# ucsdmanorlab/PSSR2

Hardware: AMD Instinct MI355X
Metric: HR tiles/sec (512^2 4xSR) train (higher is better)
Workload: dtype bf16

## Files before the change

### include/pssr_mi355.h

```cpp
#ifndef PSSR_MI355_H
#define PSSR_MI355_H

#include <stdint.h>

#ifdef __cplusplus
extern "C" {
#endif

typedef void* pssr_stream_t;

enum { PSSR_F32 = 0, PSSR_BF16 = 1, PSSR_F16 = 2 };

enum {
    PSSR_OK = 0,
    PSSR_ERR_ARG = -1,
    PSSR_ERR_LAUNCH = -2,
    PSSR_ERR_UNSUPPORTED = -3
};

int pssr_abi_version(void);
const char* pssr_last_error(void);

int pssr_pack_conv_weight(const float* w_oihw, void* packed, int cout, int cin, int ks,
                          int ci_begin, int ci_count, int mode, const int32_t* n_perm,
// ... 133 lines not shown
                                  pssr_stream_t stream);

int pssr_channel_sum_nhwc(const void* x, int cs, int co, int64_t npix, int c, double* out, int dtype,
                          pssr_stream_t stream);
int pssr_nchw_to_nhwc(const float* in, void* out, int n, int c, int64_t hw, int out_cs, float scale,
                      int dtype, pssr_stream_t stream);
int pssr_clip_u8(const float* in, uint8_t* out, int64_t n, pssr_stream_t stream);
int pssr_f64_to_f32(const double* in, float* out, int n, int accumulate, int stripes, pssr_stream_t stream);

int pssr_ssim_level_fwd(const float* x, const float* y, int planes, int h, int w, const float* win_host,
                        int k, float c1, float c2, double* sums, double* l1_sum, pssr_stream_t stream);
int pssr_avgpool2_planes(const float* in, float* out, int planes, int h, int w, pssr_stream_t stream);
int pssr_msssim_weights(const double* sums, int levels, int planes, const double* nvalid,
                        const float* level_weights, int ms, float mix, const double* l1_sum,
                        double l1_numel, const float* grad_out, float* loss_out, float* wts,
                        float* l1_coef, pssr_stream_t stream);
int pssr_ssim_level_bwd(const float* x, const float* y, int planes, int h, int w, const float* win_host,
                        int k, float c1, float c2, const float* wts, int use_ssim, const float* dcoarse,
                        int hc, int wc, const float* l1_coef, float* dx, pssr_stream_t stream);

int pssr_ssim_level_fwd_adj(const float* x, const float* y, float in_div, int planes, int h, int w, const float* win_host, int k,
                            float c1, float c2, int use_ssim, double* sums, double* l1_sum, int stripes, int64_t stripe_stride,
                            float* adj, pssr_stream_t stream);
int pssr_msssim_weights_striped(const double* sums, int stripes, int64_t stripe_stride, double* folded, int levels, int planes,
                                const double* nvalid, const float* level_weights, int ms, float mix, const double* l1_sum,
                                double l1_numel, const float* grad_out, float* loss_out, float* wts, float* l1_coef,
                                pssr_stream_t stream);
int pssr_ssim_level_bwd_adj(const float* x, const float* y, float in_div, const float* adj, int planes, int h, int w,
                            const float* win_host, int k, const float* wts, const float* dcoarse, int hc, int wc,
                            const float* l1_coef, float* dx, pssr_stream_t stream);
int pssr_avgpool2_planes_div(const float* in, float in_div, float* out, int planes, int h, int w, pssr_stream_t stream);
int pssr_avgpool2_pair_div(const float* x, const float* y, float in_div, float* xo, float* yo, int planes, int h, int w,
                           pssr_stream_t stream);

int pssr_adamw_step(float* p, const float* g, float* m, float* v, int64_t n, float lr, float beta1,
                    float beta2, float eps, float weight_decay, int64_t step, float grad_scale,
                    pssr_stream_t stream);
int pssr_adamw_step_dev(float* p, const float* g, float* m, float* v, int64_t n, int64_t* state,
                        float beta1, float beta2, float eps, float weight_decay, float grad_scale,
                        pssr_stream_t stream);
int pssr_amp_check(const float* g, int64_t n, int32_t* amp, pssr_stream_t stream);
int pssr_adamw_step_amp(float* p, const float* g, float* m, float* v, int64_t n, int64_t* state,
                        float beta1, float beta2, float eps, float weight_decay, float grad_scale,
                        int32_t* amp, float growth, float backoff, int interval, pssr_stream_t stream);

int pssr_bilinear_down_u8(const uint8_t* hr, uint8_t* tmp, uint8_t* lr, int planes, int H, int W,
                          int h, int w, pssr_stream_t stream);
int pssr_u8_to_f32(const uint8_t* in, float* out, int64_t n, pssr_stream_t stream);
int pssr_crappify_gaussian(const float* in, float* out, int tiles, int64_t per_tile, float intensity,
                           float gain, float spread, uint64_t seed, uint64_t tile_offset,
                           const double* noise, int flags, const uint64_t* tile_counter,
                           pssr_stream_t stream);
int pssr_crappify_poisson(const float* in, float* out, int tiles, int64_t per_tile, float intensity,
                          float gain, float spread, uint64_t seed, uint64_t tile_offset, int flags,
                          const uint64_t* tile_counter, pssr_stream_t stream);
int pssr_crappify_poisson_samples(const float* in, const double* samples, float* out, int64_t n, double intensity,
                                  double gain, int flags, pssr_stream_t stream);
int pssr_counter_add(uint64_t* counter, uint64_t inc, pssr_stream_t stream);
int pssr_gaussian_blur(const float* in, float* tmp, float* out, int planes, int h, int w, float sigma,
                       float gain, int flags, pssr_stream_t stream);

int pssr_crappify_saltpepper(const float* in, float* out, int tiles, int64_t per_tile, float amount, float gain, float spread,
                             uint64_t seed, uint64_t tile_offset, int flags, const uint64_t* tile_counter, pssr_stream_t stream);
int pssr_gaussian_blur_tiles(const float* in, float* tmp, float* out, int tiles, int planes_per_tile, int h, int w, float sigma,
                             float spread, float gain, uint64_t seed, uint64_t tile_offset, int flags, const uint64_t* tile_counter,
                             pssr_stream_t stream);
// ... 148 lines not shown
```

### pssr2_amd/csrc/loss.hip

```cpp
#include "common.h"

namespace {

constexpr int TS = 32;
constexpr int MAXW = 33;

struct Win { float g[MAXW]; int k; };

template <int K_DUMMY>
__global__ __launch_bounds__(256) void ssim_fwd_kernel(const float* __restrict__ X, const float* __restrict__ Y, int H, int W,
                                                       Win win, float C1, float C2, double* sums ,
                                                       double* l1_sum ) {
    extern __shared__ float lds[];
    const int k = win.k, halo = k - 1, IN = TS + halo;
    float* xs = lds;
    float* ys = xs + IN * IN;
    float* hp = ys + IN * IN;
    const int plane = blockIdx.z;
    const int oy0 = blockIdx.y * TS, ox0 = blockIdx.x * TS;
    const int VH = H - halo, VW = W - halo;
    const float* xp = X + (long)plane * H * W;
    const float* yp = Y + (long)plane * H * W;
    const int tid = threadIdx.x;
    float l1 = 0.f;
// ... 340 lines not shown
        float v[5][SEG + K - 1];
#pragma unroll
        for (int q = 0; q < 5; ++q)
#pragma unroll
            for (int j = 0; j < SEG + K - 1; ++j) v[q][j] = hp[q * IN * HPW + (r0 + j) * HPW + c];
        float m[5][SEG];
        fir_seg<K, SEG, 5>(v, win, m);
#pragma unroll
        for (int j = 0; j < SEG; ++j) {
            if (oy0 + r0 + j >= VH || ox0 + c >= VW) continue;
            const float mx = m[0][j], my = m[1][j];
            const float sxx = m[2][j] - mx * mx, syy = m[3][j] - my * my, sxy = m[4][j] - mx * my;
            const float Dcs = sxx + syy + C2;
            const float cs = (2.f * sxy + C2) / Dcs;
            const float Dl = mx * mx + my * my + C1;
            const float lum = (2.f * mx * my + C1) / Dl;
            cs_acc += cs; ss_acc += lum * cs;
        }
    }
    __shared__ float red[3][256];
    red[0][tid] = cs_acc; red[1][tid] = ss_acc; red[2][tid] = l1;
    __syncthreads();
    for (int o = 128; o > 0; o >>= 1) {
        if (tid < o) { red[0][tid] += red[0][tid + o]; red[1][tid] += red[1][tid + o]; red[2][tid] += red[2][tid + o]; }
        __syncthreads();
    }
    if (tid == 0) {
        atomicAdd(sums + plane * 2, (double)red[0][0]);
        atomicAdd(sums + plane * 2 + 1, (double)red[1][0]);
        if (l1_sum) atomicAdd(l1_sum, (double)red[2][0]);
    }
}

template <int K>
__global__ __launch_bounds__(256) void ssim_fwd_adj_k(const float* __restrict__ X, const float* __restrict__ Y, int H, int W,
                                                      Win win, float C1, float C2, double* sums, double* l1_sum, int stripes, long stripe_stride,
                                                      float* __restrict__ adj, int use_ssim, float in_mul) {
    constexpr int halo = K - 1, IN = TS + halo, SEG = 8, NS = TS / SEG;
    constexpr int HPW = TS + 1;
    extern __shared__ float lds[];
    float* xs = lds;
    float* ys = xs + IN * IN;
    float* hp = ys + IN * IN;
    const int plane = blockIdx.z;
    const int oy0 = blockIdx.y * TS, ox0 = blockIdx.x * TS;
    const int VH = H - halo, VW = W - halo;
    const float* xp = X + (long)plane * H * W;
    const float* yp = Y + (long)plane * H * W;
    const int tid = threadIdx.x;
    float l1 = 0.f;
    for (int i = tid; i < IN * IN; i += 256) {
        const int r = i / IN, c = i % IN;
        const int gy = oy0 + r, gx = ox0 + c;
        float xv = 0.f, yv = 0.f;
        if (gy < H && gx < W) { xv = __fmul_rn(xp[(long)gy * W + gx], in_mul); yv = __fmul_rn(yp[(long)gy * W + gx], in_mul); }
        xs[i] = xv; ys[i] = yv;
    }
    __syncthreads();
    if (l1_sum) {
        constexpr int r5 = K / 2;
        float wsum = 0.f;
#pragma unroll
        for (int t = 0; t < K; ++t) wsum += win.g[t];
        for (int i = tid; i < TS * TS; i += 256) {
            const int r = i / TS, c = i % TS;
            const int gy = oy0 + r, gx = ox0 + c;
            if (gy < H && gx < W) {
                float sy = wsum, sx = wsum;
                if (gy < r5 || gy >= H - r5) {
                    sy = 0.f;
#pragma unroll
                    for (int t = 0; t < K; ++t) { const int yy = gy + t - r5; if (yy >= 0 && yy < H) sy += win.g[t]; }
                }
                if (gx < r5 || gx >= W - r5) {
                    sx = 0.f;
#pragma unroll
                    for (int t = 0; t < K; ++t) { const int xx = gx + t - r5; if (xx >= 0 && xx < W) sx += win.g[t]; }
                }
                l1 += fabsf(xs[r * IN + c] - ys[r * IN + c]) * sy * sx;
            }
        }
    }
    const bool vitem = tid < TS * NS;
    const int vc = tid % TS, vr0 = (tid / TS) * SEG;
    float m[5][SEG];
#pragma unroll
    for (int q = 0; q < 5; ++q) {
        for (int it = tid; it < IN * NS; it += 256) {
            const int r = it / NS, c0 = (it % NS) * SEG;
            float v[1][SEG + K - 1];
#pragma unroll
            for (int j = 0; j < SEG + K - 1; ++j) {
                const float a = (q == 1 || q == 3) ? 0.f : xs[r * IN + c0 + j];
                const float b = (q == 0 || q == 2) ? 0.f : ys[r * IN + c0 + j];
                v[0][j] = q == 0 ? a : q == 1 ? b : q == 2 ? a * a : q == 3 ? b * b : a * b;
            }
            float o[1][SEG];
            fir_seg<K, SEG, 1>(v, win, o);
#pragma unroll
            for (int j = 0; j < SEG; ++j) hp[r * HPW + c0 + j] = o[0][j];
        }
        __syncthreads();
        if (vitem) {
            float v[1][SEG + K - 1];
#pragma unroll
            for (int j = 0; j < SEG + K - 1; ++j) v[0][j] = hp[(vr0 + j) * HPW + vc];
            float o[1][SEG];
            fir_seg<K, SEG, 1>(v, win, o);
#pragma unroll
            for (int j = 0; j < SEG; ++j) m[q][j] = o[0][j];
        }
        if (q < 4) __syncthreads();
    }
    float cs_acc = 0.f, ss_acc = 0.f;
    if (vitem) {
#pragma unroll
        for (int j = 0; j < SEG; ++j) {
            if (oy0 + vr0 + j >= VH || ox0 + vc >= VW) continue;
            const float mx = m[0][j], my = m[1][j];
            const float sxx = m[2][j] - mx * mx, syy = m[3][j] - my * my, sxy = m[4][j] - mx * my;
            const float Dcs = sxx + syy + C2;
            const float cs = (2.f * sxy + C2) / Dcs;
            const float Dl = mx * mx + my * my + C1;
            const float lum = (2.f * mx * my + C1) / Dl;
            cs_acc += cs; ss_acc += lum * cs;
            const float dcs_dmx = 2.f * (cs * mx - my) / Dcs, dcs_dexx = -cs / Dcs, dcs_dexy = 2.f / Dcs;
            float a = dcs_dmx, b = dcs_dexx, cc = dcs_dexy;
            if (use_ssim) {
                const float dl_dmx = 2.f * (my - lum * mx) / Dl;
                a = lum * dcs_dmx + cs * dl_dmx; b = lum * dcs_dexx; cc = lum * dcs_dexy;
            }
            float* ap = adj + ((long)plane * 3 * H + (oy0 + vr0 + j)) * W + ox0 + vc;
            ap[0] = a; ap[(long)H * W] = b; ap[2L * H * W] = cc;
        }
    }
    __shared__ float red[3][256];
    red[0][tid] = cs_acc; red[1][tid] = ss_acc; red[2][tid] = l1;
    __syncthreads();
    for (int o = 128; o > 0; o >>= 1) {
        if (tid < o) { red[0][tid] += red[0][tid + o]; red[1][tid] += red[1][tid + o]; red[2][tid] += red[2][tid + o]; }
        __syncthreads();
    }
    if (tid == 0) {
        const long so = (long)((blockIdx.x + blockIdx.y * 5) % stripes) * stripe_stride, lo = (long)stripes * stripe_stride;
        stat_add(sums + so + plane * 2, lo, red[0][0]);
        stat_add(sums + so + plane * 2 + 1, lo, red[1][0]);
        if (l1_sum) stat_add(l1_sum + so, lo, red[2][0]);
    }
}

template <int K>
__global__ __launch_bounds__(256) void ssim_bwd_adj_k(const float* __restrict__ X, const float* __restrict__ Y, const float* __restrict__ ADJ,
                                                      int H, int W, Win win, const float* __restrict__ wts,
                                                      const float* __restrict__ dcoarse, int HC, int WC, const float* l1_coef_p,
                                                      float* __restrict__ dX, float in_mul) {
    constexpr int halo = K - 1, AD = TS + halo;
    constexpr int SEG = 8, NS = TS / SEG;
    constexpr int ADC = AD + 1;
    constexpr int THR = AD + SEG, THW = TS + 1;
    constexpr int NL = (AD * AD + 255) / 256;
    extern __shared__ float lds[];
    float* ad = lds;
    float* th = lds + AD * ADC;
    const int plane = blockIdx.z;
    const int qy0 = blockIdx.y * TS, qx0 = blockIdx.x * TS;
    const int VH = H - halo, VW = W - halo;
    const float* xp = X + (long)plane * H * W;
    const float* yp = Y + (long)plane * H * W;
    const float* ap = ADJ + (long)plane * 3 * H * W;
    const int tid = threadIdx.x;
    const float wt = wts[plane];
    int goff[NL], lslot[NL];
#pragma unroll
    for (int u = 0; u < NL; ++u) {
        const int i = tid + u * 256;
        const int r = i / AD, c = i - r * AD;
        const int py = qy0 - halo + r, px = qx0 - halo + c;
        lslot[u] = i < AD * AD ? r * ADC + c : -1;
        goff[u] = (i < AD * AD && py >= 0 && py < VH && px >= 0 && px < VW) ? py * W + px : -1;
    }
    float pre[NL];
#define SB_LOAD(Q)                                                                                                \
    _Pragma("unroll") for (int u = 0; u < NL; ++u) pre[u] = goff[u] >= 0 ? wt * ap[(long)(Q) * H * W + goff[u]] : 0.f;
    SB_LOAD(0)
    const bool vitem = tid < TS * NS;
    const int vc = tid % TS, vr0 = (tid / TS) * SEG;
    float xv[SEG], yv[SEG], gsum[SEG];
#pragma unroll
    for (int o = 0; o < SEG; ++o) {
        const int gy = qy0 + vr0 + o, gx = qx0 + vc;
        const bool ok = vitem && gy < H && gx < W;
        xv[o] = ok ? __fmul_rn(xp[(long)gy * W + gx], in_mul) : 0.f;
        yv[o] = ok ? __fmul_rn(yp[(long)gy * W + gx], in_mul) : 0.f;
        gsum[o] = 0.f;
    }
#pragma unroll
    for (int q = 0; q < 3; ++q) {
#pragma unroll
        for (int u = 0; u < NL; ++u) if (lslot[u] >= 0) ad[lslot[u]] = pre[u];
        __syncthreads();
        if (q < 2) { SB_LOAD(q + 1) }
        for (int it = tid; it < AD * NS; it += 256) {
            const int r = it / NS, c0 = (it % NS) * SEG;
            float v[SEG + K - 1];
#pragma unroll
            for (int j = 0; j < SEG + K - 1; ++j) v[j] = ad[r * ADC + c0 + j];
#pragma unroll
            for (int o = 0; o < SEG; ++o) {
                float s_ = 0.f;
#pragma unroll
                for (int t = 0; t < K; ++t) s_ = fmaf(win.g[t], v[o + halo - t], s_);
                th[r * THW + c0 + o] = s_;
            }
        }
        __syncthreads();
        if (vitem) {
            float v[SEG + K - 1];
#pragma unroll
            for (int j = 0; j < SEG + K - 1; ++j) v[j] = th[(vr0 + j) * THW + vc];
#pragma unroll
            for (int o = 0; o < SEG; ++o) {
                float a = 0.f;
#pragma unroll
                for (int t = 0; t < K; ++t) a = fmaf(win.g[t], v[o + halo - t], a);
                if (q == 0) gsum[o] = a;
                else if (q == 1) gsum[o] = gsum[o] + 2.f * xv[o] * a;
                else gsum[o] = gsum[o] + yv[o] * a;
            }
        }
    }
#undef SB_LOAD
    if (!vitem) return;
    const float l1c = l1_coef_p ? l1_coef_p[0] : 0.f;
    constexpr int r5 = K / 2;
    float wsum = 0.f;
#pragma unroll
    for (int t = 0; t < K; ++t) wsum += win.g[t];
    float* dxp = dX + (long)plane * H * W;
#pragma unroll
    for (int o = 0; o < SEG; ++o) {
        const int gy = qy0 + vr0 + o, gx = qx0 + vc;
        if (gy >= H || gx >= W) continue;
        float g = gsum[o];
        if (dcoarse) {
            const int cy = (gy + (H & 1)) >> 1, cx = (gx + (W & 1)) >> 1;
            g += 0.25f * dcoarse[((long)plane * HC + cy) * WC + cx];
        }
        if (l1c != 0.f) {
            float sy = wsum, sx = wsum;
            if (gy < r5 || gy >= H - r5) {
                sy = 0.f;
#pragma unroll
                for (int t = 0; t < K; ++t) { const int yy = gy + t - r5; if (yy >= 0 && yy < H) sy += win.g[t]; }
            }
            if (gx < r5 || gx >= W - r5) {
                sx = 0.f;
#pragma unroll
                for (int t = 0; t < K; ++t) { const int xx = gx + t - r5; if (xx >= 0 && xx < W) sx += win.g[t]; }
            }
            const float d = xv[o] - yv[o];
            g += l1c * sy * sx * (d > 0.f ? 1.f : (d < 0.f ? -1.f : 0.f));
        }
        dxp[(long)gy * W + gx] = __fmul_rn(g, in_mul);
    }
}

template <int K>
__global__ __launch_bounds__(256, 2) void ssim_bwd_k(const float* __restrict__ X, const float* __restrict__ Y, int H, int W, Win win,
                                                  float C1, float C2, const float* __restrict__ wts, int use_ssim,
                                                  const float* __restrict__ dcoarse, int HC, int WC, const float* l1_coef_p,
                                                  float* __restrict__ dX) {
    constexpr int halo = K - 1, AD = TS + halo, IN = TS + 2 * halo;
    constexpr int SA = 7, NSA = (AD + SA - 1) / SA;
    constexpr int SEG = 8, NS = TS / SEG;
    constexpr int ADP = NSA * SA;
    extern __shared__ float lds[];
    float* xs = lds;
    constexpr int INP = IN + SA;
    float* ys = xs + IN * INP;
    float* hp = ys + IN * INP;
    float* ad = lds;
    constexpr int ADR = AD, ADC = AD;
    static_assert(3 * AD * AD <= 2 * IN * INP, "adjoint maps must fit into the input images");
    const int plane = blockIdx.z;
    const int qy0 = blockIdx.y * TS, qx0 = blockIdx.x * TS;
    const int VH = H - halo, VW = W - halo;
    const float* xp = X + (long)plane * H * W;
    const float* yp = Y + (long)plane * H * W;
    const int tid = threadIdx.x;
    const float wt = wts[plane];
    for (int i = tid; i < IN * INP; i += 256) {
        const int r = i / INP, c = i % INP;
        const int gy = qy0 - halo + r, gx = qx0 - halo + c;
        float xv = 0.f, yv = 0.f;
        if (c < IN && gy >= 0 && gy < H && gx >= 0 && gx < W) { xv = xp[(long)gy * W + gx]; yv = yp[(long)gy * W + gx]; }
        xs[i] = xv; ys[i] = yv;
    }
// ... 139 lines not shown
int pssr_ssim_level_fwd(const float* x, const float* y, int planes, int h, int w, const float* win_host, int k,
                        float c1, float c2, double* sums, double* l1_sum, pssr_stream_t s) {
    PSSR_CHECK(x && y && sums && win_host && planes > 0 && k > 0 && k <= MAXW && (k & 1), PSSR_ERR_ARG, "ssim_level_fwd: bad args");
    PSSR_CHECK(h >= k && w >= k, PSSR_ERR_ARG, "ssim_level_fwd: image %dx%d smaller than window %d", h, w, k);
    const int IN = TS + k - 1;
    const size_t lds = (size_t)(2 * IN * IN + 5 * IN * (TS + 1)) * sizeof(float);
    const int eh = l1_sum ? h : h - k + 1, ew = l1_sum ? w : w - k + 1;
    static bool attr = false;
    if (!attr) {
        (void)hipFuncSetAttribute((const void*)ssim_fwd_kernel<0>, hipFuncAttributeMaxDynamicSharedMemorySize, 160 * 1024 - 4096);
        (void)hipFuncSetAttribute((const void*)ssim_fwd_k<11>, hipFuncAttributeMaxDynamicSharedMemorySize, 160 * 1024 - 4096);
        attr = true;
    }
    if (k == 11)
        hipLaunchKernelGGL(ssim_fwd_k<11>, dim3(cdiv(ew, TS), cdiv(eh, TS), planes), dim3(256), lds, (hipStream_t)s, x, y, h, w,
                           make_win(win_host, k), c1, c2, sums, l1_sum);
    else
        hipLaunchKernelGGL(ssim_fwd_kernel<0>, dim3(cdiv(ew, TS), cdiv(eh, TS), planes), dim3(256), lds, (hipStream_t)s, x, y, h, w,
                           make_win(win_host, k), c1, c2, sums, l1_sum);
    PSSR_LAUNCH_CHECK();
    return PSSR_OK;
}

int pssr_ssim_level_fwd_adj(const float* x, const float* y, float in_div, int planes, int h, int w, const float* win_host, int k, float c1,
                            float c2, int use_ssim, double* sums, double* l1_sum, int stripes, int64_t stripe_stride, float* adj,
                            pssr_stream_t s) {
    PSSR_CHECK(x && y && sums && win_host && planes > 0 && adj && k == 11, PSSR_ERR_ARG,
               "ssim_level_fwd_adj: needs the adjoint buffer and the 11-tap window (k=%d)", k);
    PSSR_CHECK(h >= k && w >= k && stripes >= 1 && (stripes == 1 || stripe_stride > 0) && in_div > 0.f, PSSR_ERR_ARG, "ssim_level_fwd_adj: bad size / stripes / in_div");
    const int IN = TS + k - 1;
    const size_t lds = (size_t)(2 * IN * IN + IN * (TS + 1)) * sizeof(float);
    const int eh = l1_sum ? h : h - k + 1, ew = l1_sum ? w : w - k + 1;
    hipLaunchKernelGGL(ssim_fwd_adj_k<11>, dim3(cdiv(ew, TS), cdiv(eh, TS), planes), dim3(256), lds, (hipStream_t)s, x, y, h, w,
                       make_win(win_host, k), c1, c2, sums, l1_sum, stripes, (long)stripe_stride, adj, use_ssim, in_div == 1.f ? 1.f : 1.f / in_div);
    PSSR_LAUNCH_CHECK();
    return PSSR_OK;
}

int pssr_ssim_level_bwd_adj(const float* x, const float* y, float in_div, const float* adj, int planes, int h, int w, const float* win_host,
                            int k, const float* wts, const float* dcoarse, int hc, int wc, const float* l1_coef, float* dx, pssr_stream_t s) {
    PSSR_CHECK(x && y && adj && wts && dx && win_host && planes > 0 && k == 11, PSSR_ERR_ARG, "ssim_level_bwd_adj: bad args (k=%d)", k);
    constexpr int AD = TS + 10;
    const size_t lds = (size_t)(AD * (AD + 1) + (AD + 8) * (TS + 1)) * sizeof(float);
    hipLaunchKernelGGL(ssim_bwd_adj_k<11>, dim3(cdiv(w, TS), cdiv(h, TS), planes), dim3(256), lds, (hipStream_t)s, x, y, adj, h, w,
                       make_win(win_host, k), wts, dcoarse, hc, wc, l1_coef, dx, in_div == 1.f ? 1.f : 1.f / in_div);
    PSSR_LAUNCH_CHECK();
    return PSSR_OK;
}

int pssr_avgpool2_planes(const float* in, float* out, int planes, int h, int w, pssr_stream_t s) {
    return pssr_avgpool2_planes_div(in, 1.f, out, planes, h, w, s);
}

int pssr_avgpool2_planes_div(const float* in, float in_div, float* out, int planes, int h, int w, pssr_stream_t s) {
    PSSR_CHECK(in && out && planes > 0 && h > 0 && w > 0 && in_div > 0.f, PSSR_ERR_ARG, "avgpool2_planes: bad args");
    const int ho = (h + 2 * (h & 1) - 2) / 2 + 1, wo = (w + 2 * (w & 1) - 2) / 2 + 1;
    const long total = (long)planes * ho * wo;
    int blocks = (int)((total + 255) / 256); if (blocks > 8192) blocks = 8192;
    hipLaunchKernelGGL(avgpool_kernel, dim3(blocks), dim3(256), 0, (hipStream_t)s, in, out, in, out, planes, h, w, ho, wo, in_div == 1.f ? 1.f : 1.f / in_div);
    PSSR_LAUNCH_CHECK();
    return PSSR_OK;
}

int pssr_avgpool2_pair_div(const float* x, const float* y, float in_div, float* xo, float* yo, int planes, int h, int w, pssr_stream_t s) {
    PSSR_CHECK(x && y && xo && yo && planes > 0 && h > 0 && w > 0 && in_div > 0.f, PSSR_ERR_ARG, "avgpool2_pair: bad args");
    const int ho = (h + 2 * (h & 1) - 2) / 2 + 1, wo = (w + 2 * (w & 1) - 2) / 2 + 1;
    const long total = (long)planes * ho * wo;
    int blocks = (int)((total + 255) / 256); if (blocks > 8192) blocks = 8192;
    hipLaunchKernelGGL(avgpool_kernel, dim3(blocks, 2), dim3(256), 0, (hipStream_t)s, x, xo, y, yo, planes, h, w, ho, wo, in_div == 1.f ? 1.f : 1.f / in_div);
    PSSR_LAUNCH_CHECK();
    return PSSR_OK;
}

int pssr_msssim_weights(const double* sums, int levels, int planes, const double* nvalid, const float* level_weights, int ms,
                        float mix, const double* l1_sum, double l1_numel, const float* grad_out, float* loss_out, float* wts,
                        float* l1_coef, pssr_stream_t s) {
    PSSR_CHECK(sums && nvalid && loss_out && wts && l1_coef && levels > 0 && levels <= 8 && planes > 0, PSSR_ERR_ARG, "msssim_weights: bad args");
    hipLaunchKernelGGL(weights_kernel, dim3(1), dim3(256), 0, (hipStream_t)s, sums, levels, planes, nvalid, level_weights, ms, mix,
// ... 41 lines not shown
```

### pssr2_amd/ops.py

```python
from __future__ import annotations

import ctypes as C

import torch

from . import _lib as L

TORCH_DTYPE = {L.F32: torch.float32, L.BF16: torch.bfloat16, L.F16: torch.float16}


def dtype_code(dt: torch.dtype) -> int:
    if dt == torch.float32:
        return L.F32
    if dt == torch.bfloat16:
        return L.BF16
    if dt == torch.float16:
        return L.F16
    raise ValueError(f"unsupported compute dtype {dt}; use torch.float32, torch.bfloat16 or torch.float16")


def pad_to(v: int, m: int) -> int:
    return (v + m - 1) // m * m


# ... 220 lines not shown


def _win(win):
    arr = (C.c_float * len(win))(*[float(v) for v in win])
    return arr, len(win)


def ssim_level_fwd(x, y, planes, h, w, win, c1, c2, sums, l1_sum=None):
    arr, k = _win(win)
    L.check(L.lib().pssr_ssim_level_fwd(L.ptr(x), L.ptr(y), planes, h, w, arr, k, C.c_float(c1), C.c_float(c2), L.ptr(sums),
                                        L.ptr(l1_sum), L.stream_ptr()), "pssr_ssim_level_fwd")


def ssim_level_fwd_adj(x, y, planes, h, w, win, c1, c2, use_ssim, sums, l1_sum, stripes, stripe_stride, adj, in_div=1.0):
    k = len(win); arr = (C.c_float * k)(*win)
    L.check(L.lib().pssr_ssim_level_fwd_adj(L.ptr(x), L.ptr(y), C.c_float(in_div), planes, h, w, arr, k, C.c_float(c1), C.c_float(c2), int(use_ssim), L.ptr(sums),
                                            L.ptr(l1_sum), stripes, C.c_int64(stripe_stride), L.ptr(adj), L.stream_ptr()), "pssr_ssim_level_fwd_adj")


def msssim_weights_striped(sums, stripes, stripe_stride, folded, levels, planes, nvalid, level_weights, ms, mix, l1_sum, l1_numel, grad_out,
                           loss_out, wts, l1_coef):
    L.check(L.lib().pssr_msssim_weights_striped(L.ptr(sums), stripes, C.c_int64(stripe_stride), L.ptr(folded), levels, planes, L.ptr(nvalid),
                                                L.ptr(level_weights), int(ms), C.c_float(mix), L.ptr(l1_sum), C.c_double(l1_numel),
                                                L.ptr(grad_out), L.ptr(loss_out), L.ptr(wts), L.ptr(l1_coef), L.stream_ptr()),
            "pssr_msssim_weights_striped")


def ssim_level_bwd_adj(x, y, adj, planes, h, w, win, wts, dcoarse, hc, wc, l1_coef, dx, in_div=1.0):
    k = len(win); arr = (C.c_float * k)(*win)
    L.check(L.lib().pssr_ssim_level_bwd_adj(L.ptr(x), L.ptr(y), C.c_float(in_div), L.ptr(adj), planes, h, w, arr, k, L.ptr(wts), L.ptr(dcoarse), hc, wc,
                                            L.ptr(l1_coef), L.ptr(dx), L.stream_ptr()), "pssr_ssim_level_bwd_adj")


def avgpool2_planes(x, out, planes, h, w, in_div=1.0):
    L.check(L.lib().pssr_avgpool2_planes_div(L.ptr(x), C.c_float(in_div), L.ptr(out), planes, h, w, L.stream_ptr()), "pssr_avgpool2_planes_div")


def avgpool2_pair(x, y, xo, yo, planes, h, w, in_div=1.0):
    L.check(L.lib().pssr_avgpool2_pair_div(L.ptr(x), L.ptr(y), C.c_float(in_div), L.ptr(xo), L.ptr(yo), planes, h, w, L.stream_ptr()),
            "pssr_avgpool2_pair_div")


def msssim_weights(sums, levels, planes, nvalid, level_weights, ms, mix, l1_sum, l1_numel, grad_out, loss_out, wts, l1_coef):
    L.check(L.lib().pssr_msssim_weights(L.ptr(sums), levels, planes, L.ptr(nvalid), L.ptr(level_weights), int(ms), C.c_float(mix),
                                        L.ptr(l1_sum), C.c_double(l1_numel), L.ptr(grad_out), L.ptr(loss_out), L.ptr(wts),
                                        L.ptr(l1_coef), L.stream_ptr()), "pssr_msssim_weights")


def ssim_level_bwd(x, y, planes, h, w, win, c1, c2, wts, use_ssim, dcoarse, hc, wc, l1_coef, dx):
    arr, k = _win(win)
    L.check(L.lib().pssr_ssim_level_bwd(L.ptr(x), L.ptr(y), planes, h, w, arr, k, C.c_float(c1), C.c_float(c2), L.ptr(wts),
                                        int(use_ssim), L.ptr(dcoarse), hc, wc, L.ptr(l1_coef), L.ptr(dx), L.stream_ptr()),
            "pssr_ssim_level_bwd")


def adamw_step(p, g, m, v, lr, beta1, beta2, eps, weight_decay, step, grad_scale=1.0):
    L.check(L.lib().pssr_adamw_step(L.ptr(p), L.ptr(g), L.ptr(m), L.ptr(v), C.c_int64(p.numel()), C.c_float(lr), C.c_float(beta1),
                                    C.c_float(beta2), C.c_float(eps), C.c_float(weight_decay), C.c_int64(step), C.c_float(grad_scale),
                                    L.stream_ptr()), "pssr_adamw_step")


ROUND_CLIP, CLIP = 2, 1


def bilinear_down_u8(hr, h, w):
    assert hr.dtype == torch.uint8 and hr.is_cuda and hr.is_contiguous()
# ... 462 lines not shown
```

### pssr2_amd/util.py

```python
from __future__ import annotations

import inspect
import math

import numpy as np
import torch
import torch.nn as nn

from . import ops

MS_WEIGHTS = (0.0448, 0.2856, 0.3001, 0.2363, 0.1333)


def _gauss_1d(size: int, sigma: float):
    coords = torch.arange(size, dtype=torch.float) - size // 2
    g = torch.exp(-(coords ** 2) / (2 * sigma ** 2))
    return (g / g.sum()).tolist()


_CONST_CACHE = {}


class _SSIMLossFunction(torch.autograd.Function):
    @staticmethod
    def forward(ctx, x, y, cfg, in_div=1.0):
        if not x.is_cuda:
            raise RuntimeError("pssr2_amd.SSIMLoss runs on an MI355X (HIP) device only; there is no CPU fallback")
        win, mix, ms, k1, k2, data_range, lvl_w = cfg
        x = x.detach().contiguous().float()
        y = y.detach().contiguous().float()
        n, c, h, w = x.shape
        planes, k = n * c, len(win)
        levels = len(lvl_w) if ms else 1
        if ms and min(h, w) <= (k - 1) * 2 ** 4:
            raise AssertionError(f"Image size should be larger than {(k - 1) * 2 ** 4} due to the 4 downsamplings in ms-ssim")
        c1, c2 = (k1 * data_range) ** 2, (k2 * data_range) ** 2
        dev = x.device
        fused_div = in_div != 1.0 and k == 11 and ctx.needs_input_grad[0]
        if in_div != 1.0 and not fused_div:
            x, y = x / in_div, y / in_div
        div0 = in_div if fused_div else 1.0
        xs, ys, dims = [x], [y], [(h, w)]
        for lv in range(1, levels):
            hh, ww = dims[-1]
            ho, wo = (hh + 2 * (hh & 1) - 2) // 2 + 1, (ww + 2 * (ww & 1) - 2) // 2 + 1
            xo = torch.empty(planes, ho, wo, device=dev)
            yo = torch.empty(planes, ho, wo, device=dev)
            ops.avgpool2_pair(xs[-1], ys[-1], xo, yo, planes, hh, ww, div0 if lv == 1 else 1.0)
            xs.append(xo), ys.append(yo), dims.append((ho, wo))
        adjs = None
        if k == 11 and ctx.needs_input_grad[0]:
            adjs = [torch.empty(planes * 3 * hh * ww, device=dev) for hh, ww in dims]
        stripes = 16 if adjs is not None else 1
        sstride = levels * planes * 2 + 2
        rows = 2 * stripes if stripes > 1 else 1
        sums = torch.zeros(rows * sstride + (sstride if stripes > 1 else 0), dtype=torch.float64, device=dev)
        l1_sum = sums[sstride - 2:sstride - 1] if mix < 1 else None
        for l in range(levels):
            hh, ww = dims[l]
            if adjs is not None:
                ops.ssim_level_fwd_adj(xs[l], ys[l], planes, hh, ww, win, c1, c2, l == levels - 1, sums[l * planes * 2:],
                                       l1_sum if l == 0 else None, stripes, sstride, adjs[l], div0 if l == 0 else 1.0)
            else:
                ops.ssim_level_fwd(xs[l], ys[l], planes, hh, ww, win, c1, c2, sums[l * planes * 2:], l1_sum if l == 0 else None)
        ckey = (tuple(dims), k, tuple(lvl_w) if ms else (1.0,), str(dev))
        cached = _CONST_CACHE.get(ckey)
        if cached is None:
            cached = _CONST_CACHE[ckey] = (
                torch.tensor([float((hh - k + 1) * (ww - k + 1)) for hh, ww in dims], dtype=torch.float64, device=dev),
                torch.tensor(list(lvl_w) if ms else [1.0], dtype=torch.float32, device=dev))
        nvalid, lw = cached
        loss = torch.empty(1, dtype=torch.float32, device=dev)
        wts = torch.empty(levels * planes, dtype=torch.float32, device=dev)
        l1c = torch.empty(1, dtype=torch.float32, device=dev)
        if stripes > 1:
            ops.msssim_weights_striped(sums, stripes, sstride, sums[rows * sstride:], levels, planes, nvalid, lw, ms, mix, l1_sum, float(x.numel()),
                                       None, loss, wts, l1c)
            sums = sums[rows * sstride:]
            l1_sum = sums[levels * planes * 2:levels * planes * 2 + 1] if l1_sum is not None else None
        else:
            ops.msssim_weights(sums, levels, planes, nvalid, lw, ms, mix, l1_sum, float(x.numel()), None, loss, wts, l1c)
        ctx.saved = (xs, ys, dims, sums, nvalid, lw, l1_sum, cfg, planes, x.shape, adjs, div0, in_div if not fused_div else 1.0)
        return loss[0]

    @staticmethod
    def backward(ctx, grad_out):
        xs, ys, dims, sums, nvalid, lw, l1_sum, cfg, planes, shape, adjs, div0, post_div = ctx.saved
        win, mix, ms, k1, k2, data_range, lvl_w = cfg
        levels = len(xs)
        dev = xs[0].device
        c1, c2 = (k1 * data_range) ** 2, (k2 * data_range) ** 2
        go = grad_out.detach().float().reshape(1).contiguous()
        loss = torch.empty(1, dtype=torch.float32, device=dev)
        wts = torch.empty(levels * planes, dtype=torch.float32, device=dev)
        l1c = torch.empty(1, dtype=torch.float32, device=dev)
        ops.msssim_weights(sums, levels, planes, nvalid, lw, ms, mix, l1_sum, float(xs[0].numel()), go, loss, wts, l1c)
        dcoarse, hc, wc = None, 0, 0
        for l in range(levels - 1, -1, -1):
            hh, ww = dims[l]
            dx = torch.empty(planes, hh, ww, device=dev)
            use_ssim = (l == levels - 1)
            l1_arg = l1c if (l == 0 and l1_sum is not None) else None
            if adjs is not None:
                ops.ssim_level_bwd_adj(xs[l], ys[l], adjs[l], planes, hh, ww, win, wts[l * planes:], dcoarse, hc, wc, l1_arg, dx,
                                       div0 if l == 0 else 1.0)
            else:
                ops.ssim_level_bwd(xs[l], ys[l], planes, hh, ww, win, c1, c2, wts[l * planes:], use_ssim, dcoarse, hc, wc, l1_arg, dx)
            dcoarse, hc, wc = dx, hh, ww
        g = dcoarse.view(shape)
        if post_div != 1.0:
            g = g / post_div
        return g, None, None, None


class SSIMLoss(nn.Module):
    def __init__(self, channels: int = 1, mix: float = .8, win_size: int = 11, win_sigma: float = 1.5, ms: bool = True, kwargs=None):
        super().__init__()
        kwargs = {} if kwargs is None else dict(kwargs)
        if win_size % 2 != 1:
            raise ValueError("Window size should be odd.")
        self.K = tuple(kwargs.pop("K", (0.01, 0.03)))
        self.weights = tuple(kwargs.pop("weights", None) or MS_WEIGHTS)
        if kwargs:
            raise TypeError(f"unsupported pytorch_msssim options on the MI355X path: {sorted(kwargs)}")
        self.win = _gauss_1d(win_size, win_sigma)
        self.channels, self.win_size, self.mix, self.ms = channels, win_size, mix, ms

    def forward(self, input, target):
        if input.shape != target.shape:
            raise ValueError(f"Input images should have the same dimensions, but got {input.shape} and {target.shape}.")
        cfg = (self.win, float(self.mix), bool(self.ms), self.K[0], self.K[1], 1.0, self.weights)
# ... 171 lines not shown
```

Measured before the change: 2392.

## Batch MS-SSIM pyramid levels into fused launches with in-kernel downsampling

Level 0 of the MS-SSIM forward now writes all four downsampled pyramid levels from its shared-memory tile, so the separate avgpool launches are dropped. Levels 1-4 run in one launch that uses a per-block level table, in both forward and backward. The backward coarse-gradient chain is folded into the level-0 backward kernel rather than done level by level. This cuts kernel launches and serial dependencies in the loss, in exchange for extra per-block work, added register and LDS pressure, and shape restrictions (multiples of 16, 11-tap window).

```diff
diff --git a/include/pssr_mi355.h b/include/pssr_mi355.h
--- a/include/pssr_mi355.h
+++ b/include/pssr_mi355.h
@@ -189,6 +189,24 @@
 int pssr_avgpool2_planes_div(const float* in, float in_div, float* out, int planes, int h, int w, pssr_stream_t stream);
 int pssr_avgpool2_pair_div(const float* x, const float* y, float in_div, float* xo, float* yo, int planes, int h, int w,
                            pssr_stream_t stream);
+
+struct pssr_ssim_level {
+    const float* x; const float* y;
+    float* adj;
+    float* dx;
+    int h, w;
+};
+int pssr_ssim_level0_fwd_pyr(const float* x, const float* y, float in_div, int planes, int h, int w, const float* win_host, int k,
+                             float c1, float c2, double* sums, double* l1_sum, int stripes, int64_t stripe_stride, float* adj,
+                             float* const* pyr_x, float* const* pyr_y, pssr_stream_t stream);
+int pssr_ssim_levels_fwd_adj(const struct pssr_ssim_level* levels, int n, int first_level, int last_is_ssim, int planes,
+                             const float* win_host, int k, float c1, float c2, double* sums, int stripes, int64_t stripe_stride,
+                             pssr_stream_t stream);
+int pssr_ssim_levels_bwd_adj(const struct pssr_ssim_level* levels, int n, int first_level, int planes, const float* win_host, int k,
+                             const float* wts, pssr_stream_t stream);
+int pssr_ssim_level0_bwd_chain(const float* x, const float* y, float in_div, const float* adj, int planes, int h, int w,
+                               const float* win_host, int k, const float* wts, const float* const* g, const float* l1_coef,
+                               float* dx, pssr_stream_t stream);
 
 int pssr_adamw_step(float* p, const float* g, float* m, float* v, int64_t n, float lr, float beta1,
                     float beta2, float eps, float weight_decay, int64_t step, float grad_scale,
diff --git a/pssr2_amd/csrc/loss.hip b/pssr2_amd/csrc/loss.hip
--- a/pssr2_amd/csrc/loss.hip
+++ b/pssr2_amd/csrc/loss.hip
@@ -396,18 +396,44 @@
     }
 }
 
+struct Pyr { float* x[4]; float* y[4]; };
+
+__device__ __forceinline__ float pool4(float a, float b, float c, float d) {
+    float s = __fadd_rn(0.f, a);
+    s = __fadd_rn(s, b); s = __fadd_rn(s, c); s = __fadd_rn(s, d);
+    return __fmul_rn(0.25f, s);
+}
+
+template <int L>
+__device__ __forceinline__ float pyr_val(const float* l1, int i, int j) {
+    if constexpr (L == 1) return l1[i * (TS / 2) + j];
+    else return pool4(pyr_val<L - 1>(l1, 2 * i, 2 * j), pyr_val<L - 1>(l1, 2 * i, 2 * j + 1),
+                      pyr_val<L - 1>(l1, 2 * i + 1, 2 * j), pyr_val<L - 1>(l1, 2 * i + 1, 2 * j + 1));
+}
+
+template <int L>
+__device__ __forceinline__ void pyr_store(const Pyr& pyr, const float* l1, int map, int pos, int plane, int oy0, int ox0, int H, int W) {
+    constexpr int N = TS >> L;
+    const int i = pos / N, j = pos % N;
+    const int HL = H >> L, WL = W >> L, gy = (oy0 >> L) + i, gx = (ox0 >> L) + j;
+    if (gy >= HL || gx >= WL) return;
+    float* dst = map ? pyr.y[L - 1] : pyr.x[L - 1];
+    dst[((long)plane * HL + gy) * WL + gx] = pyr_val<L>(l1, i, j);
+}
+
 template <int K>
-__global__ __launch_bounds__(256) void ssim_fwd_adj_k(const float* __restrict__ X, const float* __restrict__ Y, int H, int W,
-                                                      Win win, float C1, float C2, double* sums, double* l1_sum, int stripes, long stripe_stride,
-                                                      float* __restrict__ adj, int use_ssim, float in_mul) {
+__device__ __forceinline__ void ssim_fwd_adj_tile(const float* __restrict__ X, const float* __restrict__ Y, int H, int W,
+                                                  const Win& win, float C1, float C2, double* sums, double* l1_sum, int stripes, long stripe_stride,
+                                                  float* __restrict__ adj, int use_ssim, float in_mul, const Pyr& pyr,
+                                                  int bx, int by, int plane) {
     constexpr int halo = K - 1, IN = TS + halo, SEG = 8, NS = TS / SEG;
     constexpr int HPW = TS + 1;
     extern __shared__ float lds[];
+    __shared__ float red[3][256];
     float* xs = lds;
     float* ys = xs + IN * IN;
     float* hp = ys + IN * IN;
-    const int plane = blockIdx.z;
-    const int oy0 = blockIdx.y * TS, ox0 = blockIdx.x * TS;
+    const int oy0 = by * TS, ox0 = bx * TS;
     const int VH = H - halo, VW = W - halo;
     const float* xp = X + (long)plane * H * W;
     const float* yp = Y + (long)plane * H * W;
@@ -421,6 +447,18 @@
         xs[i] = xv; ys[i] = yv;
     }
     __syncthreads();
+    if (pyr.x[0]) {
+        const int i = tid / (TS / 2), j = tid % (TS / 2);
+        const float* a = xs + 2 * i * IN + 2 * j;
+        const float* b = ys + 2 * i * IN + 2 * j;
+        const float px = pool4(a[0], a[1], a[IN], a[IN + 1]), py = pool4(b[0], b[1], b[IN], b[IN + 1]);
+        red[0][tid] = px; red[1][tid] = py;
+        const int H1 = H >> 1, W1 = W >> 1, gy = (oy0 >> 1) + i, gx = (ox0 >> 1) + j;
+        if (gy < H1 && gx < W1) {
+            pyr.x[0][((long)plane * H1 + gy) * W1 + gx] = px;
+            pyr.y[0][((long)plane * H1 + gy) * W1 + gx] = py;
+        }
+    }
     if (l1_sum) {
         constexpr int r5 = K / 2;
         float wsum = 0.f;
@@ -465,6 +503,12 @@
             for (int j = 0; j < SEG; ++j) hp[r * HPW + c0 + j] = o[0][j];
         }
         __syncthreads();
+        if (q == 0 && pyr.x[0] && !vitem) {
+            const int t = tid - TS * NS;
+            pyr_store<2>(pyr, red[t >> 6], t >> 6, t & 63, plane, oy0, ox0, H, W);
+            if (t < 32) pyr_store<3>(pyr, red[t >> 4], t >> 4, t & 15, plane, oy0, ox0, H, W);
+            else if (t < 40) pyr_store<4>(pyr, red[(t - 32) >> 2], (t - 32) >> 2, t & 3, plane, oy0, ox0, H, W);
+        }
         if (vitem) {
             float v[1][SEG + K - 1];
 #pragma unroll
@@ -498,7 +542,6 @@
             ap[0] = a; ap[(long)H * W] = b; ap[2L * H * W] = cc;
         }
     }
-    __shared__ float red[3][256];
     red[0][tid] = cs_acc; red[1][tid] = ss_acc; red[2][tid] = l1;
     __syncthreads();
     for (int o = 128; o > 0; o >>= 1) {
@@ -506,7 +549,7 @@
         __syncthreads();
     }
     if (tid == 0) {
-        const long so = (long)((blockIdx.x + blockIdx.y * 5) % stripes) * stripe_stride, lo = (long)stripes * stripe_stride;
+        const long so = (long)((bx + by * 5) % stripes) * stripe_stride, lo = (long)stripes * stripe_stride;
         stat_add(sums + so + plane * 2, lo, red[0][0]);
         stat_add(sums + so + plane * 2 + 1, lo, red[1][0]);
         if (l1_sum) stat_add(l1_sum + so, lo, red[2][0]);
@@ -514,10 +557,40 @@
 }
 
 template <int K>
-__global__ __launch_bounds__(256) void ssim_bwd_adj_k(const float* __restrict__ X, const float* __restrict__ Y, const float* __restrict__ ADJ,
-                                                      int H, int W, Win win, const float* __restrict__ wts,
-                                                      const float* __restrict__ dcoarse, int HC, int WC, const float* l1_coef_p,
-                                                      float* __restrict__ dX, float in_mul) {
+__global__ __launch_bounds__(256) void ssim_fwd_adj_k(const float* __restrict__ X, const float* __restrict__ Y, int H, int W,
+                                                      Win win, float C1, float C2, double* sums, double* l1_sum, int stripes, long stripe_stride,
+                                                      float* __restrict__ adj, int use_ssim, float in_mul, Pyr pyr) {
+    ssim_fwd_adj_tile<K>(X, Y, H, W, win, C1, C2, sums, l1_sum, stripes, stripe_stride, adj, use_ssim, in_mul, pyr,
+                         blockIdx.x, blockIdx.y, blockIdx.z);
+}
+
+struct LevelDesc { const float* x; const float* y; const float* adj_in; float* out; int H, W, slot, use_ssim, first, tiles_x; };
+struct LevelTable { LevelDesc l[4]; int n; };
+
+__device__ __forceinline__ LevelDesc pick_level(const LevelTable& tab, int b) {
+    LevelDesc d = tab.l[0];
+#pragma unroll
+    for (int i = 1; i < 4; ++i) if (i < tab.n && b >= tab.l[i].first) d = tab.l[i];
+    return d;
+}
+
+template <int K>
+__global__ __launch_bounds__(256) void ssim_fwd_adj_levels_k(LevelTable tab, Win win, float C1, float C2, double* sums, int stripes,
+                                                             long stripe_stride) {
+    const LevelDesc d = pick_level(tab, blockIdx.x);
+    const int t = blockIdx.x - d.first;
+    const Pyr none = {};
+    ssim_fwd_adj_tile<K>(d.x, d.y, d.H, d.W, win, C1, C2, sums + d.slot, nullptr, stripes, stripe_stride, d.out, d.use_ssim, 1.f, none,
+                         t % d.tiles_x, t / d.tiles_x, blockIdx.z);
+}
+
+struct Chain { const float* g[4]; };
+
+template <int K>
+__device__ __forceinline__ void ssim_bwd_adj_tile(const float* __restrict__ X, const float* __restrict__ Y, const float* __restrict__ ADJ,
+                                                  int H, int W, const Win& win, const float* __restrict__ wts,
+                                                  const float* __restrict__ dcoarse, int HC, int WC, const Chain& chain,
+                                                  const float* l1_coef_p, float* __restrict__ dX, float in_mul, int bx, int by, int plane) {
     constexpr int halo = K - 1, AD = TS + halo;
     constexpr int SEG = 8, NS = TS / SEG;
     constexpr int ADC = AD + 1;
@@ -526,8 +599,7 @@
     extern __shared__ float lds[];
     float* ad = lds;
     float* th = lds + AD * ADC;
-    const int plane = blockIdx.z;
-    const int qy0 = blockIdx.y * TS, qx0 = blockIdx.x * TS;
+    const int qy0 = by * TS, qx0 = bx * TS;
     const int VH = H - halo, VW = W - halo;
     const float* xp = X + (long)plane * H * W;
     const float* yp = Y + (long)plane * H * W;
@@ -558,6 +630,18 @@
         yv[o] = ok ? __fmul_rn(yp[(long)gy * W + gx], in_mul) : 0.f;
         gsum[o] = 0.f;
     }
+    float d1[SEG / 2] = {0.f, 0.f, 0.f, 0.f};
+    if (chain.g[0] && vitem && qy0 + vr0 < H && qx0 + vc < W) {
+        const int gy = qy0 + vr0, gx = qx0 + vc;
+        const int H1 = H >> 1, W1 = W >> 1, H2 = H >> 2, W2 = W >> 2, H3 = H >> 3, W3 = W >> 3, H4 = H >> 4, W4 = W >> 4;
+        const float d4 = chain.g[3][((long)plane * H4 + (gy >> 4)) * W4 + (gx >> 4)];
+        const float d3 = fmaf(0.25f, d4, chain.g[2][((long)plane * H3 + (gy >> 3)) * W3 + (gx >> 3)]);
+        float d2[2];
+#pragma unroll
+        for (int a = 0; a < 2; ++a) d2[a] = fmaf(0.25f, d3, chain.g[1][((long)plane * H2 + (gy >> 2) + a) * W2 + (gx >> 2)]);
+#pragma unroll
+        for (int b = 0; b < SEG / 2; ++b) d1[b] = fmaf(0.25f, d2[b >> 1], chain.g[0][((long)plane * H1 + (gy >> 1) + b) * W1 + (gx >> 1)]);
+    }
 #pragma unroll
     for (int q = 0; q < 3; ++q) {
 #pragma unroll
@@ -608,8 +692,9 @@
         float g = gsum[o];
         if (dcoarse) {
             const int cy = (gy + (H & 1)) >> 1, cx = (gx + (W & 1)) >> 1;
-            g += 0.25f * dcoarse[((long)plane * HC + cy) * WC + cx];
-        }
+            g = fmaf(0.25f, dcoarse[((long)plane * HC + cy) * WC + cx], g);
+        }
+        if (chain.g[0]) g = fmaf(0.25f, d1[o >> 1], g);
         if (l1c != 0.f) {
             float sy = wsum, sx = wsum;
             if (gy < r5 || gy >= H - r5) {
@@ -627,6 +712,23 @@
         }
         dxp[(long)gy * W + gx] = __fmul_rn(g, in_mul);
     }
+}
+
+template <int K>
+__global__ __launch_bounds__(256) void ssim_bwd_adj_k(const float* __restrict__ X, const float* __restrict__ Y, const float* __restrict__ ADJ,
+                                                      int H, int W, Win win, const float* __restrict__ wts,
+                                                      const float* __restrict__ dcoarse, int HC, int WC, Chain chain, const float* l1_coef_p,
+                                                      float* __restrict__ dX, float in_mul) {
+    ssim_bwd_adj_tile<K>(X, Y, ADJ, H, W, win, wts, dcoarse, HC, WC, chain, l1_coef_p, dX, in_mul, blockIdx.x, blockIdx.y, blockIdx.z);
+}
+
+template <int K>
+__global__ __launch_bounds__(256) void ssim_bwd_adj_levels_k(LevelTable tab, Win win, const float* __restrict__ wts) {
+    const LevelDesc d = pick_level(tab, blockIdx.x);
+    const int t = blockIdx.x - d.first;
+    const Chain none = {};
+    ssim_bwd_adj_tile<K>(d.x, d.y, d.adj_in, d.H, d.W, win, wts + d.slot, nullptr, 0, 0, none, nullptr, d.out, 1.f,
+                         t % d.tiles_x, t / d.tiles_x, blockIdx.z);
 }
 
 template <int K>
@@ -832,7 +934,95 @@
     const size_t lds = (size_t)(2 * IN * IN + IN * (TS + 1)) * sizeof(float);
     const int eh = l1_sum ? h : h - k + 1, ew = l1_sum ? w : w - k + 1;
     hipLaunchKernelGGL(ssim_fwd_adj_k<11>, dim3(cdiv(ew, TS), cdiv(eh, TS), planes), dim3(256), lds, (hipStream_t)s, x, y, h, w,
-                       make_win(win_host, k), c1, c2, sums, l1_sum, stripes, (long)stripe_stride, adj, use_ssim, in_div == 1.f ? 1.f : 1.f / in_div);
+                       make_win(win_host, k), c1, c2, sums, l1_sum, stripes, (long)stripe_stride, adj, use_ssim, in_div == 1.f ? 1.f : 1.f / in_div,
+                       Pyr{});
+    PSSR_LAUNCH_CHECK();
+    return PSSR_OK;
+}
+
+int pssr_ssim_level0_fwd_pyr(const float* x, const float* y, float in_div, int planes, int h, int w, const float* win_host, int k, float c1,
+                             float c2, double* sums, double* l1_sum, int stripes, int64_t stripe_stride, float* adj,
+                             float* const* pyr_x, float* const* pyr_y, pssr_stream_t s) {
+    PSSR_CHECK(x && y && sums && win_host && planes > 0 && adj && k == 11 && pyr_x && pyr_y, PSSR_ERR_ARG,
+               "ssim_level0_fwd_pyr: needs the adjoint buffer, the pyramid tables and the 11-tap window (k=%d)", k);
+    PSSR_CHECK(stripes >= 1 && (stripes == 1 || stripe_stride > 0) && in_div > 0.f, PSSR_ERR_ARG, "ssim_level0_fwd_pyr: bad stripes / in_div");
+    PSSR_CHECK(h % 16 == 0 && w % 16 == 0 && (h >> 4) >= k && (w >> 4) >= k, PSSR_ERR_ARG,
+               "ssim_level0_fwd_pyr: %dx%d is not a multiple of 16 with a level-4 map of at least the window", h, w);
+    Pyr pyr;
+    for (int i = 0; i < 4; ++i) {
+        PSSR_CHECK(pyr_x[i] && pyr_y[i], PSSR_ERR_ARG, "ssim_level0_fwd_pyr: null pyramid level %d", i + 1);
+        pyr.x[i] = pyr_x[i]; pyr.y[i] = pyr_y[i];
+    }
+    const int IN = TS + k - 1;
+    const size_t lds = (size_t)(2 * IN * IN + IN * (TS + 1)) * sizeof(float);
+    hipLaunchKernelGGL(ssim_fwd_adj_k<11>, dim3(cdiv(w, TS), cdiv(h, TS), planes), dim3(256), lds, (hipStream_t)s, x, y, h, w,
+                       make_win(win_host, k), c1, c2, sums, l1_sum, stripes, (long)stripe_stride, adj, 0, in_div == 1.f ? 1.f : 1.f / in_div, pyr);
+    PSSR_LAUNCH_CHECK();
+    return PSSR_OK;
+}
+
+static int make_level_table(const pssr_ssim_level* lv, int n, int first_level, int k, int slot_stride, bool backward, LevelTable* tab) {
+    int blocks = 0;
+    tab->n = n;
+    for (int i = 0; i < 4; ++i) {
+        LevelDesc& d = tab->l[i];
+        if (i >= n) { d = tab->l[0]; d.first = 0x7fffffff; continue; }
+        const pssr_ssim_level& L = lv[i];
+        if (!(L.x && L.y && L.adj && (!backward || L.dx) && L.h >= k && L.w >= k)) return -1;
+        d.x = L.x; d.y = L.y; d.adj_in = L.adj; d.out = backward ? L.dx : L.adj;
+        d.H = L.h; d.W = L.w; d.slot = (first_level + i) * slot_stride; d.use_ssim = 0;
+        d.first = blocks;
+        const int ew = backward ? L.w : L.w - k + 1, eh = backward ? L.h : L.h - k + 1;
+        d.tiles_x = cdiv(ew, TS);
+        blocks += d.tiles_x * cdiv(eh, TS);
+    }
+    return blocks;
+}
+
+int pssr_ssim_levels_fwd_adj(const pssr_ssim_level* levels, int n, int first_level, int last_is_ssim, int planes, const float* win_host,
+                             int k, float c1, float c2, double* sums, int stripes, int64_t stripe_stride, pssr_stream_t s) {
+    PSSR_CHECK(levels && n >= 1 && n <= 4 && first_level >= 0 && sums && win_host && planes > 0 && k == 11, PSSR_ERR_ARG,
+               "ssim_levels_fwd_adj: 1-4 levels and the 11-tap window (n=%d, k=%d)", n, k);
+    PSSR_CHECK(stripes >= 1 && (stripes == 1 || stripe_stride > 0), PSSR_ERR_ARG, "ssim_levels_fwd_adj: bad stripes");
+    LevelTable tab;
+    const int blocks = make_level_table(levels, n, first_level, k, planes * 2, false, &tab);
+    PSSR_CHECK(blocks > 0, PSSR_ERR_ARG, "ssim_levels_fwd_adj: null pointer or a level smaller than the window");
+    if (last_is_ssim) tab.l[n - 1].use_ssim = 1;
+    const int IN = TS + k - 1;
+    const size_t lds = (size_t)(2 * IN * IN + IN * (TS + 1)) * sizeof(float);
+    hipLaunchKernelGGL(ssim_fwd_adj_levels_k<11>, dim3(blocks, 1, planes), dim3(256), lds, (hipStream_t)s, tab, make_win(win_host, k), c1, c2,
+                       sums, stripes, (long)stripe_stride);
+    PSSR_LAUNCH_CHECK();
+    return PSSR_OK;
+}
+
+int pssr_ssim_levels_bwd_adj(const pssr_ssim_level* levels, int n, int first_level, int planes, const float* win_host, int k,
+                             const float* wts, pssr_stream_t s) {
+    PSSR_CHECK(levels && n >= 1 && n <= 4 && first_level >= 0 && wts && win_host && planes > 0 && k == 11, PSSR_ERR_ARG,
+               "ssim_levels_bwd_adj: 1-4 levels and the 11-tap window (n=%d, k=%d)", n, k);
+    LevelTable tab;
+    const int blocks = make_level_table(levels, n, first_level, k, planes, true, &tab);
+    PSSR_CHECK(blocks > 0, PSSR_ERR_ARG, "ssim_levels_bwd_adj: null pointer or a level smaller than the window");
+    constexpr int AD = TS + 10;
+    const size_t lds = (size_t)(AD * (AD + 1) + (AD + 8) * (TS + 1)) * sizeof(float);
+    hipLaunchKernelGGL(ssim_bwd_adj_levels_k<11>, dim3(blocks, 1, planes), dim3(256), lds, (hipStream_t)s, tab, make_win(win_host, k), wts);
+    PSSR_LAUNCH_CHECK();
+    return PSSR_OK;
+}
+
+int pssr_ssim_level0_bwd_chain(const float* x, const float* y, float in_div, const float* adj, int planes, int h, int w, const float* win_host,
+                               int k, const float* wts, const float* const* g, const float* l1_coef, float* dx, pssr_stream_t s) {
+    PSSR_CHECK(x && y && adj && wts && dx && win_host && planes > 0 && k == 11 && g, PSSR_ERR_ARG, "ssim_level0_bwd_chain: bad args (k=%d)", k);
+    PSSR_CHECK(h % 16 == 0 && w % 16 == 0 && in_div > 0.f, PSSR_ERR_ARG, "ssim_level0_bwd_chain: %dx%d is not a multiple of 16", h, w);
+    Chain chain;
+    for (int i = 0; i < 4; ++i) {
+        PSSR_CHECK(g[i], PSSR_ERR_ARG, "ssim_level0_bwd_chain: null gradient of level %d", i + 1);
+        chain.g[i] = g[i];
+    }
+    constexpr int AD = TS + 10;
+    const size_t lds = (size_t)(AD * (AD + 1) + (AD + 8) * (TS + 1)) * sizeof(float);
+    hipLaunchKernelGGL(ssim_bwd_adj_k<11>, dim3(cdiv(w, TS), cdiv(h, TS), planes), dim3(256), lds, (hipStream_t)s, x, y, adj, h, w,
+                       make_win(win_host, k), wts, (const float*)nullptr, 0, 0, chain, l1_coef, dx, in_div == 1.f ? 1.f : 1.f / in_div);
     PSSR_LAUNCH_CHECK();
     return PSSR_OK;
 }
@@ -843,7 +1033,7 @@
     constexpr int AD = TS + 10;
     const size_t lds = (size_t)(AD * (AD + 1) + (AD + 8) * (TS + 1)) * sizeof(float);
     hipLaunchKernelGGL(ssim_bwd_adj_k<11>, dim3(cdiv(w, TS), cdiv(h, TS), planes), dim3(256), lds, (hipStream_t)s, x, y, adj, h, w,
-                       make_win(win_host, k), wts, dcoarse, hc, wc, l1_coef, dx, in_div == 1.f ? 1.f : 1.f / in_div);
+                       make_win(win_host, k), wts, dcoarse, hc, wc, Chain{}, l1_coef, dx, in_div == 1.f ? 1.f : 1.f / in_div);
     PSSR_LAUNCH_CHECK();
     return PSSR_OK;
 }
diff --git a/pssr2_amd/ops.py b/pssr2_amd/ops.py
--- a/pssr2_amd/ops.py
+++ b/pssr2_amd/ops.py
@@ -276,6 +276,48 @@
                                             L.ptr(l1_coef), L.ptr(dx), L.stream_ptr()), "pssr_ssim_level_bwd_adj")
 
 
+class _SsimLevel(C.Structure):
+    _fields_ = [("x", C.c_void_p), ("y", C.c_void_p), ("adj", C.c_void_p), ("dx", C.c_void_p), ("h", C.c_int), ("w", C.c_int)]
+
+
+def _ptr_table(tensors):
+    return (C.c_void_p * len(tensors))(*[t.data_ptr() for t in tensors])
+
+
+def _level_table(xs, ys, adjs, dxs, dims):
+    tab = (_SsimLevel * len(xs))()
+    for i, (x, y, a, (h, w)) in enumerate(zip(xs, ys, adjs, dims)):
+        tab[i].x, tab[i].y, tab[i].adj, tab[i].h, tab[i].w = x.data_ptr(), y.data_ptr(), a.data_ptr(), h, w
+        tab[i].dx = dxs[i].data_ptr() if dxs is not None else None
+    return tab
+
+
+def ssim_level0_fwd_pyr(x, y, planes, h, w, win, c1, c2, sums, l1_sum, stripes, stripe_stride, adj, pyr_x, pyr_y, in_div=1.0):
+    k = len(win); arr = (C.c_float * k)(*win)
+    L.check(L.lib().pssr_ssim_level0_fwd_pyr(L.ptr(x), L.ptr(y), C.c_float(in_div), planes, h, w, arr, k, C.c_float(c1), C.c_float(c2), L.ptr(sums),
+                                             L.ptr(l1_sum), stripes, C.c_int64(stripe_stride), L.ptr(adj), _ptr_table(pyr_x), _ptr_table(pyr_y),
+                                             L.stream_ptr()), "pssr_ssim_level0_fwd_pyr")
+
+
+def ssim_levels_fwd_adj(xs, ys, adjs, dims, first_level, last_is_ssim, planes, win, c1, c2, sums, stripes, stripe_stride):
+    k = len(win); arr = (C.c_float * k)(*win)
+    L.check(L.lib().pssr_ssim_levels_fwd_adj(_level_table(xs, ys, adjs, None, dims), len(xs), first_level, int(last_is_ssim), planes, arr, k,
+                                             C.c_float(c1), C.c_float(c2), L.ptr(sums), stripes, C.c_int64(stripe_stride), L.stream_ptr()),
+            "pssr_ssim_levels_fwd_adj")
+
+
+def ssim_levels_bwd_adj(xs, ys, adjs, dxs, dims, first_level, planes, win, wts):
+    k = len(win); arr = (C.c_float * k)(*win)
+    L.check(L.lib().pssr_ssim_levels_bwd_adj(_level_table(xs, ys, adjs, dxs, dims), len(xs), first_level, planes, arr, k, L.ptr(wts),
+                                             L.stream_ptr()), "pssr_ssim_levels_bwd_adj")
+
+
+def ssim_level0_bwd_chain(x, y, adj, planes, h, w, win, wts, gs, l1_coef, dx, in_div=1.0):
+    k = len(win); arr = (C.c_float * k)(*win)
+    L.check(L.lib().pssr_ssim_level0_bwd_chain(L.ptr(x), L.ptr(y), C.c_float(in_div), L.ptr(adj), planes, h, w, arr, k, L.ptr(wts), _ptr_table(gs),
+                                               L.ptr(l1_coef), L.ptr(dx), L.stream_ptr()), "pssr_ssim_level0_bwd_chain")
+
+
 def avgpool2_planes(x, out, planes, h, w, in_div=1.0):
     L.check(L.lib().pssr_avgpool2_planes_div(L.ptr(x), C.c_float(in_div), L.ptr(out), planes, h, w, L.stream_ptr()), "pssr_avgpool2_planes_div")
 
diff --git a/pssr2_amd/util.py b/pssr2_amd/util.py
--- a/pssr2_amd/util.py
+++ b/pssr2_amd/util.py
@@ -19,6 +19,7 @@
 
 
 _CONST_CACHE = {}
+_LOSS_BATCH = __import__("os").environ.get("PSSR_LOSS_BATCH", "1") != "0"
 
 
 class _SSIMLossFunction(torch.autograd.Function):
@@ -40,13 +41,15 @@
         if in_div != 1.0 and not fused_div:
             x, y = x / in_div, y / in_div
         div0 = in_div if fused_div else 1.0
+        batched = _LOSS_BATCH and ms and levels == 5 and k == 11 and ctx.needs_input_grad[0] and h % 16 == 0 and w % 16 == 0
         xs, ys, dims = [x], [y], [(h, w)]
         for lv in range(1, levels):
             hh, ww = dims[-1]
             ho, wo = (hh + 2 * (hh & 1) - 2) // 2 + 1, (ww + 2 * (ww & 1) - 2) // 2 + 1
             xo = torch.empty(planes, ho, wo, device=dev)
             yo = torch.empty(planes, ho, wo, device=dev)
-            ops.avgpool2_pair(xs[-1], ys[-1], xo, yo, planes, hh, ww, div0 if lv == 1 else 1.0)
+            if not batched:
+                ops.avgpool2_pair(xs[-1], ys[-1], xo, yo, planes, hh, ww, div0 if lv == 1 else 1.0)
             xs.append(xo), ys.append(yo), dims.append((ho, wo))
         adjs = None
         if k == 11 and ctx.needs_input_grad[0]:
@@ -56,7 +59,10 @@
         rows = 2 * stripes if stripes > 1 else 1
         sums = torch.zeros(rows * sstride + (sstride if stripes > 1 else 0), dtype=torch.float64, device=dev)
         l1_sum = sums[sstride - 2:sstride - 1] if mix < 1 else None
-        for l in range(levels):
+        if batched:
+            ops.ssim_level0_fwd_pyr(x, y, planes, h, w, win, c1, c2, sums, l1_sum, stripes, sstride, adjs[0], xs[1:], ys[1:], div0)
+            ops.ssim_levels_fwd_adj(xs[1:], ys[1:], adjs[1:], dims[1:], 1, True, planes, win, c1, c2, sums, stripes, sstride)
+        for l in range(0 if not batched else levels, levels):
             hh, ww = dims[l]
             if adjs is not None:
                 ops.ssim_level_fwd_adj(xs[l], ys[l], planes, hh, ww, win, c1, c2, l == levels - 1, sums[l * planes * 2:],
@@ -80,12 +86,12 @@
             l1_sum = sums[levels * planes * 2:levels * planes * 2 + 1] if l1_sum is not None else None
         else:
             ops.msssim_weights(sums, levels, planes, nvalid, lw, ms, mix, l1_sum, float(x.numel()), None, loss, wts, l1c)
-        ctx.saved = (xs, ys, dims, sums, nvalid, lw, l1_sum, cfg, planes, x.shape, adjs, div0, in_div if not fused_div else 1.0)
+        ctx.saved = (xs, ys, dims, sums, nvalid, lw, l1_sum, cfg, planes, x.shape, adjs, div0, in_div if not fused_div else 1.0, batched)
         return loss[0]
 
     @staticmethod
     def backward(ctx, grad_out):
-        xs, ys, dims, sums, nvalid, lw, l1_sum, cfg, planes, shape, adjs, div0, post_div = ctx.saved
+        xs, ys, dims, sums, nvalid, lw, l1_sum, cfg, planes, shape, adjs, div0, post_div, batched = ctx.saved
         win, mix, ms, k1, k2, data_range, lvl_w = cfg
         levels = len(xs)
         dev = xs[0].device
@@ -96,7 +102,12 @@
         l1c = torch.empty(1, dtype=torch.float32, device=dev)
         ops.msssim_weights(sums, levels, planes, nvalid, lw, ms, mix, l1_sum, float(xs[0].numel()), go, loss, wts, l1c)
         dcoarse, hc, wc = None, 0, 0
-        for l in range(levels - 1, -1, -1):
+        if batched:
+            gs = [torch.empty(planes, hh, ww, device=dev) for hh, ww in dims[1:]]
+            ops.ssim_levels_bwd_adj(xs[1:], ys[1:], adjs[1:], gs, dims[1:], 1, planes, win, wts)
+            dcoarse = torch.empty(planes, *dims[0], device=dev)
+            ops.ssim_level0_bwd_chain(xs[0], ys[0], adjs[0], planes, *dims[0], win, wts, gs, l1c if l1_sum is not None else None, dcoarse, div0)
+        for l in range(levels - 1 if not batched else -1, -1, -1):
             hh, ww = dims[l]
             dx = torch.empty(planes, hh, ww, device=dev)
             use_ssim = (l == levels - 1)
```

After: 2415 (median of 5 runs). About the same (+1.0%).
